# sanweiliti/LEMO

Hardware: AMD Instinct MI355X
Metric: fitting-iterations/sec (T=120 frames) (higher is better)
Workload: dtype f32

## Files before the change

lemo_amd/csrc/conv_pair_kernels.hip:

```cpp
#include "conv_common.hpp"
#include "conv_f16.hpp"

namespace lemo {

constexpr int CP_TH = 10, CP_TW = 14;
constexpr int CP_INW = CP_TW + 4, CP_INH = CP_TH + 4, CP_NIN = CP_INW * CP_INH;
constexpr int CP_MIDW = CP_TW + 2, CP_MIDH = CP_TH + 2, CP_NMID = CP_MIDW * CP_MIDH;
constexpr int CP_MIDP = CP_MIDW + 2, CP_NMIDP = CP_MIDP * CP_MIDH;
constexpr int CP_NOUT = CP_TH * CP_TW;
constexpr int CP_PL_IN = CP_NIN * 16, CP_GRP_IN = 2 * CP_PL_IN;
constexpr int CP_PL_MID = CP_NMIDP * 16, CP_GRP_MID = 2 * CP_PL_MID;
constexpr int CP_MID_OFF = 8 * CP_GRP_IN;
constexpr int CP_WMAX_OFF = CP_MID_OFF + 8 * CP_GRP_MID;
constexpr int CP_SMEM = CP_WMAX_OFF + 3 * 8 * 4;
constexpr int CP_NSLOT = 4;
static_assert(CP_MIDW == 16 && CP_NMID == 6 * 32 && CP_INW == CP_MIDP, "N-tiles = 2 rows x 16 columns on grids of row pitch 18");
static_assert(4 * 2 * CP_NIN <= CP_NSLOT * 512 && CP_NOUT == 140, "staging slots");
static_assert(8 * 6 * 256 * 4 <= CP_MID_OFF, "the K-half exchange (6 quads per wave) fits the dead input planes");

struct PairArgs {
  const float* in;
  const uint4* wA;
  const uint4* wB;
  const float *biasA, *biasB;
  const float *auxA, *auxB;
  float* mid;
  float* out;
  float winvA, winvB;
  int H, W, ntx, ntiles;
  unsigned long long* dbg;
};

template <int NT> struct PairSplit {
  static constexpr int NQ = NT == 3 ? 6 : 4;
  static constexpr int keep_tile(int KH, int i) { return i < 4 ? KH : 2; }
  static constexpr int keep_quad(int KH, int i) { return i < 4 ? i : (i - 4) + 2 * KH; }
  static constexpr int give_tile(int KH, int i) { return i < 4 ? 1 - KH : 2; }
  static constexpr int give_quad(int KH, int i) { return i < 4 ? i : (i - 4) + 2 * (1 - KH); }
};

template <int NT, int KH>
__device__ __forceinline__ void pair_exchange(const f32x16 (&acc)[3], float4 (&v)[6], float* red_mine, const float* red_theirs) {
  typedef PairSplit<NT> S;
#pragma unroll
  for (int i = 0; i < S::NQ; ++i) {
    const int t = S::give_tile(KH, i), q = S::give_quad(KH, i);
    st4(red_mine + i * 256, make_float4(acc[t][4 * q], acc[t][4 * q + 1], acc[t][4 * q + 2], acc[t][4 * q + 3]));
  }
  __syncthreads();
#pragma unroll
  for (int i = 0; i < S::NQ; ++i) {
    const int t = S::keep_tile(KH, i), q = S::keep_quad(KH, i);
    const float4 o = ld4(red_theirs + i * 256);
    const float4 m = make_float4(acc[t][4 * q], acc[t][4 * q + 1], acc[t][4 * q + 2], acc[t][4 * q + 3]);
    v[i] = KH ? make_float4(o.x + m.x, o.y + m.y, o.z + m.z, o.w + m.w) : make_float4(m.x + o.x, m.y + o.y, m.z + o.z, m.w + o.w);
  }
}

__device__ __forceinline__ int cp_lane_col(int j) { return j < 16 ? j : ((j - 18) & 15); }

#define CP_RA 3

__device__ __forceinline__ void pair_preload_a(uint4 (&ra)[CP_RA][2], const uint4* __restrict__ w, int kh, int ch, int lane) {
#pragma unroll
  for (int u0 = 0; u0 < CP_RA - 1; ++u0)
#pragma unroll
    for (int s_ = 0; s_ < 2; ++s_) ra[u0][s_] = w[(unsigned)((((2 * kh) * 9 + u0) * 2 + ch) * 2 + s_) * 64u + lane];
}

template <int NT, int GRP, int PL, int PITCH, typename MidFn, typename EndFn>
__device__ __forceinline__ void pair_kloop(f32x16 (&acc)[3], uint4 (&ra)[CP_RA][2], const uint4* __restrict__ w, const unsigned char* bbase,
                                           const int (&li)[3], int kh, int ch, int lane, MidFn&& mid_fn, EndFn&& end_fn) {
  const int h = lane >> 5;
  uint4 rb[2][3][2];
#define CP_LOAD_A(SET, U)                                                                              \
  _Pragma("unroll") for (int s_ = 0; s_ < 2; ++s_)                                                     \
    ra[SET][s_] = w[(unsigned)((((2 * kh + (U) / 9) * 9 + (U) % 9) * 2 + ch) * 2 + s_) * 64u + lane];
#define CP_LOAD_B(SET, U)                                                                              \
  _Pragma("unroll") for (int nt_ = 0; nt_ < NT; ++nt_)                                                 \
    _Pragma("unroll") for (int s_ = 0; s_ < 2; ++s_)                                                   \
      rb[SET][nt_][s_] = *reinterpret_cast<const uint4*>(                                              \
          bbase + (2 * (2 * kh + (U) / 9) + h) * GRP + s_ * PL + (li[nt_] + (((U) % 9) / 3 - 1) * PITCH + (((U) % 9) % 3 - 1)) * 16);
#define CP_MFMA1(SA, SETA, SB, SETB)                                                                   \
  _Pragma("unroll") for (int nt_ = 0; nt_ < NT; ++nt_)                                                 \
    acc[nt_] = __builtin_amdgcn_mfma_f32_32x32x16_f16(__builtin_bit_cast(f16x8, ra[SETA][SA]),         \
                                                      __builtin_bit_cast(f16x8, rb[SETB][nt_][SB]), acc[nt_], 0, 0, 0);
#pragma unroll
  for (int cc = 0; cc < 2; ++cc) {
    CP_LOAD_B((cc * 9) & 1, cc * 9)
#pragma unroll
    for (int tap = 0; tap < 9; ++tap) {
      const int u = cc * 9 + tap;
      if (u + CP_RA - 1 < 18) { CP_LOAD_A((u + CP_RA - 1) % CP_RA, u + CP_RA - 1) }
      if (tap + 1 < 9) { CP_LOAD_B((u + 1) & 1, u + 1) }
      __builtin_amdgcn_sched_barrier(0);
      CP_MFMA1(0, u % CP_RA, 1, u & 1) CP_MFMA1(1, u % CP_RA, 0, u & 1) CP_MFMA1(0, u % CP_RA, 0, u & 1)
      mid_fn(cc, tap);
      __builtin_amdgcn_sched_barrier(0);
    }
    end_fn(cc);
  }
#undef CP_LOAD_A
#undef CP_LOAD_B
#undef CP_MFMA1
}

template <int EPI, int NT>
__device__ __forceinline__ void pair_layer2(const PairArgs& a, unsigned char* smem, float* smem_f, int y0, int x0, int T0, int ng2, int ch,
                                            int kh, int lane, float smi, uint4 (&ra)[CP_RA][2]) {
  const int j = lane & 31, h = lane >> 5;
  const int Wp = a.W + 2, HWp = (a.H + 2) * Wp;
  int lo[3] = {0, 0, 0}, poff[3] = {0, 0, 0};
  bool ok[3] = {false, false, false};
#pragma unroll
  for (int nt = 0; nt < NT; ++nt) {
    const int oy = 2 * (T0 + nt) + (j >> 4), c = cp_lane_col(j), ox = c - 1;
    lo[nt] = (oy + 1) * CP_MIDP + c + 1;
    const int y = y0 + oy, x = x0 + ox;
    ok[nt] = ox >= 0 && ox < CP_TW && y < a.H && x < a.W;
    const int yc = y < a.H ? y : a.H - 1, xc = x < 0 ? 0 : (x < a.W ? x : a.W - 1);
    poff[nt] = (yc + 1) * Wp + (xc + 1);
  }
  f32x16 acc[3];
#pragma unroll
  for (int nt = 0; nt < 3; ++nt)
#pragma unroll
    for (int r = 0; r < 16; ++r) acc[nt][r] = 0.f;
  pair_kloop<NT, CP_GRP_MID, CP_PL_MID, CP_MIDP>(acc, ra, a.wB, smem + CP_MID_OFF, lo, kh, ch, lane, [](int, int) {}, [](int) {});
  {
    const float f = smi * a.winvB;
#pragma unroll
    for (int nt = 0; nt < NT; ++nt)
#pragma unroll
      for (int r = 0; r < 16; ++r) acc[nt][r] *= f;
  }
  typedef PairSplit<NT> S;
  const int KHu = __builtin_amdgcn_readfirstlane(kh);
  const int poA = KHu ? poff[1] : poff[0], poB = poff[2];
  const bool okA = KHu ? ok[1] : ok[0], okB = ok[2];
  float4 eo[6];
#pragma unroll
  for (int i = 0; i < S::NQ; ++i) {
    const int q = KHu ? S::keep_quad(1, i) : S::keep_quad(0, i);
    const int c0 = ch * 32 + q * 8 + 4 * h;
    const int po = i < 4 ? poA : poB;
    eo[i] = EPI == 1 ? ld4(a.auxB + ((size_t)(c0 >> 3) * HWp + po) * 8 + (c0 & 7)) : ld4(a.biasB + c0);
  }
  float* red = smem_f + ((ng2 * 2 + ch) * 2) * 1536 + lane * 4;
  float4 v[6];
  if (KHu) pair_exchange<NT, 1>(acc, v, red + 1536, red);
  else pair_exchange<NT, 0>(acc, v, red, red + 1536);
#pragma unroll
  for (int i = 0; i < S::NQ; ++i) {
    const int q = KHu ? S::keep_quad(1, i) : S::keep_quad(0, i);
    const int c0 = ch * 32 + q * 8 + 4 * h;
    const int po = i < 4 ? poA : poB;
    const bool st = i < 4 ? okA : okB;
    float4 r = v[i];
    if (EPI == 1) {
      r.x *= lrelu_grad_from_out(eo[i].x); r.y *= lrelu_grad_from_out(eo[i].y);
      r.z *= lrelu_grad_from_out(eo[i].z); r.w *= lrelu_grad_from_out(eo[i].w);
    } else {
      r.x = lrelu(r.x + eo[i].x); r.y = lrelu(r.y + eo[i].y); r.z = lrelu(r.z + eo[i].z); r.w = lrelu(r.w + eo[i].w);
    }
    if (st) st4(a.out + ((size_t)(c0 >> 3) * HWp + po) * 8 + (c0 & 7), r);
  }
}

template <int EPI, bool DBG>
__global__ void __launch_bounds__(512)
conv3x3_pair_kernel(PairArgs a) {
  unsigned long long t_start = 0, t_pro = 0, t_l1 = 0, t_mid = 0, t_ex = 0, t_mx = 0;
  if (DBG) t_start = __builtin_amdgcn_s_memtime();
  LEMO_DYN_SMEM(smem_f);
  unsigned char* smem = reinterpret_cast<unsigned char*>(smem_f);
  float* wmax = reinterpret_cast<float*>(smem + CP_WMAX_OFF);
  const int tid = (int)threadIdx.x, lane = tid & 63, wave = tid >> 6;
  const int j = lane & 31, h = lane >> 5;
  const int ng = wave & 1, ch = (wave >> 1) & 1, kh = wave >> 2;
  const int H = a.H, W = a.W, Wp = W + 2, HWp = (H + 2) * Wp;
  const unsigned in_gstride = (unsigned)HWp * 8u;
  int tile = (int)blockIdx.x;
  {
    const int q = a.ntiles >> 3, r = a.ntiles & 7, xcd = tile & 7, k = tile >> 3;
    tile = (xcd < r ? xcd * (q + 1) : r * (q + 1) + (xcd - r) * q) + k;
  }
  const int ty = tile / a.ntx, tx = tile - ty * a.ntx;
  const int y0 = ty * CP_TH, x0 = tx * CP_TW;

  uint4 ra[CP_RA][2];
  pair_preload_a(ra, a.wA, kh, ch, lane);

  unsigned offB[CP_NSLOT];
  int dstB[CP_NSLOT];
#pragma unroll
  for (int k = 0; k < CP_NSLOT; ++k) {
    int c0 = tid + k * 512;
    c0 = c0 < 4 * 2 * CP_NIN ? c0 : 4 * 2 * CP_NIN - 1;
    const int gg = c0 / (2 * CP_NIN), c = c0 - gg * (2 * CP_NIN);
    const int px = c >> 1, half = c & 1;
    const int r = px / CP_INW, col = px - r * CP_INW;
    int gy = y0 - 2 + r, gx = x0 - 2 + col;
    gy = (gy < -1 ? -1 : (gy > H ? H : gy)) + 1;
    gx = (gx < -1 ? -1 : (gx > W ? W : gx)) + 1;
    const int g0 = (gg >> 1) * 4 + (gg & 1);
    offB[k] = (unsigned)g0 * in_gstride + (unsigned)(gy * Wp + gx) * 8u + 4u * half;
    dstB[k] = g0 * CP_GRP_IN + px * 16 + 8 * half;
  }
  float4 stB[CP_NSLOT];
#pragma unroll
  for (int k = 0; k < CP_NSLOT; ++k) stB[k] = ld4(a.in + offB[k]);
  if (tid < CP_MIDH * 2 * 16) {
    const int pl = tid / (CP_MIDH * 2), rc = tid - pl * (CP_MIDH * 2);
    *reinterpret_cast<uint4*>(smem + CP_MID_OFF + pl * CP_PL_MID + ((rc >> 1) * CP_MIDP + (rc & 1) * (CP_MIDP - 1)) * 16) = make_uint4(0u, 0u, 0u, 0u);
  }
  float sc[2] = {1.f, 1.f}, sci[2] = {1.f, 1.f};
  {
    float m = 0.f;
#pragma unroll
    for (int k = 0; k < CP_NSLOT; ++k) m = absmax4(stB[k], m);
    m = wave_max(m);
    if (lane == 0) wmax[wave] = m;
    __syncthreads();
    float mm = 0.f;
#pragma unroll
    for (int i = 0; i < 8; ++i) mm = fmaxf(mm, wmax[i]);
    f16_scale_for(mm, sc[0], sci[0]);
  }
#pragma unroll
  for (int k = 0; k < CP_NSLOT; ++k) {
    uint2 s0, s1;
    split2x4(stB[k], sc[0], s0, s1);
    *reinterpret_cast<uint2*>(smem + dstB[k]) = s0;
    *reinterpret_cast<uint2*>(smem + dstB[k] + CP_PL_IN) = s1;
  }
#pragma unroll
  for (int k = 0; k < CP_NSLOT; ++k) stB[k] = ld4(a.in + 2u * in_gstride + offB[k]);
  __syncthreads();
  if (DBG) t_pro = __builtin_amdgcn_s_memtime();

  int li[3];
#pragma unroll
  for (int nt = 0; nt < 3; ++nt) {
    const int my = 2 * (3 * ng + nt) + (j >> 4), mx = cp_lane_col(j);
    li[nt] = (my + 1) * CP_INW + mx + 1;
  }
  f32x16 acc[3];
#pragma unroll
  for (int nt = 0; nt < 3; ++nt)
#pragma unroll
    for (int r = 0; r < 16; ++r) acc[nt][r] = 0.f;
  pair_kloop<3, CP_GRP_IN, CP_PL_IN, CP_INW>(
      acc, ra, a.wA, smem, li, kh, ch, lane,
      [&](int cc, int tap) {
        if (cc != 0) return;
        if (tap == 0) {
          float m = 0.f;
#pragma unroll
          for (int k = 0; k < CP_NSLOT; ++k) m = absmax4(stB[k], m);
          m = wave_max(m);
          if (lane == 0) wmax[8 + wave] = m;
        }
        if (tap == 1) {
          __syncthreads();
          float mm = 0.f;
#pragma unroll
          for (int i = 0; i < 8; ++i) mm = fmaxf(mm, wmax[8 + i]);
          f16_scale_after(mm, sc[0], sc[1], sci[1]);
        }
#pragma unroll
        for (int k = 0; k < CP_NSLOT; ++k) {
          if (2 + (7 * k) / CP_NSLOT != tap) continue;
          uint2 s0, s1;
          split2x4(stB[k], sc[1], s0, s1);
          *reinterpret_cast<uint2*>(smem + 2 * CP_GRP_IN + dstB[k]) = s0;
          *reinterpret_cast<uint2*>(smem + 2 * CP_GRP_IN + dstB[k] + CP_PL_IN) = s1;
        }
      },
      [&](int cc) {
        __syncthreads();
        if (cc == 0) {
          const float f = sc[1] * sci[0];
#pragma unroll
          for (int nt = 0; nt < 3; ++nt)
#pragma unroll
            for (int r = 0; r < 16; ++r) acc[nt][r] *= f;
        }
      });
  if (DBG) t_l1 = __builtin_amdgcn_s_memtime();
  pair_preload_a(ra, a.wB, kh, ch, lane);
  {
    const float f = sci[1] * a.winvA;
#pragma unroll
    for (int nt = 0; nt < 3; ++nt)
#pragma unroll
      for (int r = 0; r < 16; ++r) acc[nt][r] *= f;
  }

  const int KHu = __builtin_amdgcn_readfirstlane(kh);
  typedef PairSplit<3> S3;
  int mp0, mp1, mpoff0, mpoff1;
  bool inimg0, inimg1, inner0, inner1;
  {
    auto geom = [&](int t, int& p_, int& poff_, bool& inimg_, bool& inner_) {
      const int my = 2 * (3 * ng + t) + (j >> 4), mx = cp_lane_col(j);
      const int y = y0 - 1 + my, x = x0 - 1 + mx;
      p_ = my * CP_MIDP + mx + 1;
      inimg_ = (unsigned)y < (unsigned)H && (unsigned)x < (unsigned)W;
      inner_ = inimg_ && my >= 1 && my <= CP_TH && mx >= 1 && mx <= CP_TW;
      const int yc = y < 0 ? 0 : (y >= H ? H - 1 : y), xc = x < 0 ? 0 : (x >= W ? W - 1 : x);
      poff_ = (yc + 1) * Wp + (xc + 1);
    };
    geom(KHu, mp0, mpoff0, inimg0, inner0);
    geom(2, mp1, mpoff1, inimg1, inner1);
  }
  float4 eo[6];
#pragma unroll
  for (int i = 0; i < 6; ++i) {
    const int q = KHu ? S3::keep_quad(1, i) : S3::keep_quad(0, i);
    const int c0 = ch * 32 + q * 8 + 4 * h;
    const int po = i < 4 ? mpoff0 : mpoff1;
    eo[i] = EPI == 1 ? ld4(a.auxA + ((size_t)(c0 >> 3) * HWp + po) * 8 + (c0 & 7)) : ld4(a.biasA + c0);
  }
  float4 v[6];
  {
    float* red = smem_f + ((ng * 2 + ch) * 2) * 1536 + lane * 4;
    if (KHu) pair_exchange<3, 1>(acc, v, red + 1536, red);
    else pair_exchange<3, 0>(acc, v, red, red + 1536);
  }
  if (DBG) t_ex = __builtin_amdgcn_s_memtime();
  float mloc = 0.f;
#pragma unroll
  for (int i = 0; i < 6; ++i) {
    const bool in_i = i < 4 ? inimg0 : inimg1;
    float4 r = v[i];
    if (EPI == 1) {
      r.x *= lrelu_grad_from_out(eo[i].x); r.y *= lrelu_grad_from_out(eo[i].y);
      r.z *= lrelu_grad_from_out(eo[i].z); r.w *= lrelu_grad_from_out(eo[i].w);
    } else {
      r.x = lrelu(r.x + eo[i].x); r.y = lrelu(r.y + eo[i].y); r.z = lrelu(r.z + eo[i].z); r.w = lrelu(r.w + eo[i].w);
    }
    if (!in_i) r = make_float4(0.f, 0.f, 0.f, 0.f);
    v[i] = r;
    mloc = absmax4(r, mloc);
  }
  mloc = wave_max(mloc);
  if (lane == 0) wmax[16 + wave] = mloc;
  __syncthreads();
  float sm, smi;
  {
    float mm = 0.f;
#pragma unroll
    for (int i = 0; i < 8; ++i) mm = fmaxf(mm, wmax[16 + i]);
    f16_scale_for(mm, sm, smi);
  }
  if (DBG) t_mx = __builtin_amdgcn_s_memtime();
#pragma unroll
  for (int i = 0; i < 6; ++i) {
    const int q = KHu ? S3::keep_quad(1, i) : S3::keep_quad(0, i);
    uint2 s0, s1;
    split2x4(v[i], sm, s0, s1);
    unsigned char* d = smem + CP_MID_OFF + (ch * 4 + q) * CP_GRP_MID + (i < 4 ? mp0 : mp1) * 16 + 8 * h;
    *reinterpret_cast<uint2*>(d) = s0;
    *reinterpret_cast<uint2*>(d + CP_PL_MID) = s1;
  }
  __syncthreads();
  if (DBG) t_mid = __builtin_amdgcn_s_memtime();

  const int ng2 = __builtin_amdgcn_readfirstlane(ng ^ kh);
  if (ng2) pair_layer2<EPI, 2>(a, smem, smem_f, y0, x0, 3, 1, ch, kh, lane, smi, ra);
  else pair_layer2<EPI, 3>(a, smem, smem_f, y0, x0, 0, 0, ch, kh, lane, smi, ra);
  if (EPI != 1) {
#pragma unroll
    for (int i = 0; i < 6; ++i) {
      const int q = KHu ? S3::keep_quad(1, i) : S3::keep_quad(0, i);
      const int c0 = ch * 32 + q * 8 + 4 * h;
      if (i < 4 ? inner0 : inner1) st4(a.mid + ((size_t)(c0 >> 3) * HWp + (i < 4 ? mpoff0 : mpoff1)) * 8 + (c0 & 7), v[i]);
    }
  }
  if (DBG && lane == 0) {
    unsigned long long* r = a.dbg + ((size_t)blockIdx.x * 8 + wave) * 8;
    r[0] = __builtin_amdgcn_s_getreg(63492);
    r[1] = t_ex;
    r[2] = t_start; r[3] = __builtin_amdgcn_s_memtime(); r[4] = t_pro; r[5] = t_l1; r[6] = t_mid; r[7] = t_mx;
  }
}

int conv_pair_init() {
  static LdsOptinOnce once;
  return lds_optin(once, {{&conv3x3_pair_kernel<0, false>, CP_SMEM}, {&conv3x3_pair_kernel<1, false>, CP_SMEM}, {&conv3x3_pair_kernel<0, true>, CP_SMEM}});
}

bool conv3x3_pair_supported(int H, int W, int c0, int c1, int c2) {
  return c0 == 64 && c1 == 64 && c2 == 64 && H >= 1 && W >= 1 && (long)H * W <= (1l << 24);
}

int conv3x3_pair_f16(const float* in, const void* wA, float winvA, const float* biasA, const float* auxA, float* mid, const void* wB,
                     float winvB, const float* biasB, const float* auxB, float* out, int H, int W, int epi, hipStream_t s,
                     unsigned long long* dbg) {
  if (!conv3x3_pair_supported(H, W, 64, 64, 64) || (epi != 0 && epi != 1)) return LEMO_ERR_SHAPE;
  if (!in || !wA || !wB || !out || !(winvA > 0.f) || !(winvB > 0.f)) return LEMO_ERR_ARG;
  if (epi == 0 ? (!biasA || !biasB || !mid) : (!auxA || !auxB)) return LEMO_ERR_ARG;
  if (dbg && epi != 0) return LEMO_ERR_ARG;
  if (int rc = conv_pair_init()) return rc;
  PairArgs a{};
  a.in = in; a.wA = reinterpret_cast<const uint4*>(wA); a.wB = reinterpret_cast<const uint4*>(wB);
  a.biasA = biasA; a.biasB = biasB; a.auxA = auxA; a.auxB = auxB; a.mid = mid; a.out = out;
  a.winvA = winvA; a.winvB = winvB; a.H = H; a.W = W;
  a.ntx = (W + CP_TW - 1) / CP_TW;
  a.ntiles = a.ntx * ((H + CP_TH - 1) / CP_TH);
  a.dbg = dbg;
  if (dbg) hipLaunchKernelGGL((conv3x3_pair_kernel<0, true>), dim3(a.ntiles), dim3(512), CP_SMEM, s, a);
  else if (epi == 0) hipLaunchKernelGGL((conv3x3_pair_kernel<0, false>), dim3(a.ntiles), dim3(512), CP_SMEM, s, a);
  else hipLaunchKernelGGL((conv3x3_pair_kernel<1, false>), dim3(a.ntiles), dim3(512), CP_SMEM, s, a);
  return (int)hipGetLastError();
}

}
```

lemo_amd/priors.py:

```python
from __future__ import annotations

import ctypes as C
from typing import Dict, List

import numpy as np
import torch
import torch.nn as nn

from . import _hip
from ._hip import ptr

ENC_CHANNELS = [1, 32, 32, 64, 64, 64, 64, 64, 64, 64, 64]
"""models/AE_sep.py:77-89 with z_channel=64: channels before/after each of the 10 conv layers."""


def enc_layer_keys() -> List[str]:
    return [f'enc_blc{b}.main.{i}' for b in range(1, 6) for i in (0, 2)]


def pack_conv3x3(w: np.ndarray) -> np.ndarray:
    co, ci = w.shape[:2]
    assert ci % 8 == 0
    t = w.reshape(co, ci // 8, 8, 9)
    return np.ascontiguousarray(t.transpose(3, 1, 0, 2), np.float32)


def pack_conv3x3_bwd(w: np.ndarray) -> np.ndarray:
    wf = w[:, :, ::-1, ::-1].transpose(1, 0, 2, 3)
    return pack_conv3x3(np.ascontiguousarray(wf))


def pack_conv3x3_gmajor(w: np.ndarray) -> np.ndarray:
    return np.ascontiguousarray(pack_conv3x3(w).transpose(1, 0, 2, 3))


def pack_conv3x3_bwd_gmajor(w: np.ndarray) -> np.ndarray:
    return np.ascontiguousarray(pack_conv3x3_bwd(w).transpose(1, 0, 2, 3))


def bf16_round(x: np.ndarray) -> np.ndarray:
    u = np.ascontiguousarray(x, np.float32).view(np.uint32).astype(np.uint64)
    r = ((u + 0x7FFF + ((u >> 16) & 1)) >> 16) << 16
    return r.astype(np.uint32).view(np.float32)


def bf16_split3(x: np.ndarray):
    x = np.ascontiguousarray(x, np.float32)
    hi = bf16_round(x)
    r1 = x - hi
    mid = bf16_round(r1)
    lo = bf16_round(r1 - mid)
    assert np.array_equal(hi.astype(np.float64) + mid.astype(np.float64) + lo.astype(np.float64), x.astype(np.float64))
    return hi, mid, lo


def pack_conv3x3_split(w: np.ndarray) -> np.ndarray:
    co, ci = w.shape[:2]
    assert ci % 16 == 0 and co % 32 == 0
    pieces = np.stack(bf16_split3(w), 0)
    bits = (pieces.view(np.uint32) >> 16).astype(np.uint16)
    t = bits.reshape(3, co // 32, 32, ci // 16, 2, 8, 9)
    t = t.transpose(3, 6, 1, 0, 4, 2, 5)
    return np.ascontiguousarray(t).reshape(ci // 16, 9, co // 32, 3, 64, 8)


def pack_conv3x3_bwd_split(w: np.ndarray) -> np.ndarray:
    wf = w[:, :, ::-1, ::-1].transpose(1, 0, 2, 3)
    return pack_conv3x3_split(np.ascontiguousarray(wf))


def f16_split2(x: np.ndarray):
    x = np.ascontiguousarray(x, np.float32)
    m = float(np.abs(x).max())
    k = 14 - int(np.floor(np.log2(m))) if m > 0 else 0
    xs = x * np.float32(2.0 ** k)
    hi = xs.astype(np.float16)
    lo = (xs - hi.astype(np.float32)).astype(np.float16)
    assert np.isfinite(hi).all()
    return hi, lo, float(2.0 ** -k)


def pack_conv3x3_split_f16(w: np.ndarray):
    co, ci = w.shape[:2]
    assert ci % 16 == 0 and co % 32 == 0
    hi, lo, winv = f16_split2(w)
    bits = np.stack([hi, lo], 0).view(np.uint16)
    t = bits.reshape(2, co // 32, 32, ci // 16, 2, 8, 9)
    t = t.transpose(3, 6, 1, 0, 4, 2, 5)
    return np.ascontiguousarray(t).reshape(ci // 16, 9, co // 32, 2, 64, 8), winv


def pack_conv3x3_bwd_split_f16(w: np.ndarray):
    wf = w[:, :, ::-1, ::-1].transpose(1, 0, 2, 3)
    return pack_conv3x3_split_f16(np.ascontiguousarray(wf))


WINO_VARIANT = 10
_WINO_G = np.array([[1.0, 0.0, 0.0], [0.5, 0.5, 0.5], [0.5, -0.5, 0.5], [0.0, 0.0, 1.0]], np.float64)


def pack_conv3x3_wino_f16(w: np.ndarray):
    co, ci = w.shape[:2]
    assert co == 64 and ci == 64 and w.shape[2:] == (3, 3)
    U = np.einsum('ij,ocjk,lk->ocil', _WINO_G, np.asarray(w, np.float64), _WINO_G).reshape(co, ci, 16)
    m = float(np.abs(U).max())
    k = 14 - int(np.floor(np.log2(m))) if m > 0 else 0
    xs = U * 2.0 ** k
    hi = xs.astype(np.float16)
    lo = (xs - hi.astype(np.float64)).astype(np.float16)
    assert np.isfinite(hi).all()
    bits = np.stack([hi, lo], 0).view(np.uint16)
    t = bits.reshape(2, co // 32, 32, ci // 16, 2, 8, 16)
    t = t.transpose(6, 3, 1, 0, 4, 2, 5)
    return np.ascontiguousarray(t).reshape(16, ci // 16, co // 32, 2, 64, 8), float(2.0 ** -k)


def pack_conv3x3_bwd_wino_f16(w: np.ndarray):
    wf = w[:, :, ::-1, ::-1].transpose(1, 0, 2, 3)
    return pack_conv3x3_wino_f16(np.ascontiguousarray(wf))


def cg8p_alloc(C_: int, H: int, W: int, device) -> torch.Tensor:
    return torch.zeros(max(C_ // 8, 1), (H + 2) * (W + 2), 8, dtype=torch.float32, device=device)


def to_cg8p(x: torch.Tensor) -> torch.Tensor:
    Cn, H, W = x.shape
    buf = torch.zeros(Cn // 8, H + 2, W + 2, 8, dtype=torch.float32, device=x.device)
    buf[:, 1:-1, 1:-1, :] = x.reshape(Cn // 8, 8, H, W).permute(0, 2, 3, 1)
    return buf.reshape(Cn // 8, (H + 2) * (W + 2), 8).contiguous()


def from_cg8p(buf: torch.Tensor, H: int, W: int) -> torch.Tensor:
    G = buf.shape[0]
    return buf.reshape(G, H + 2, W + 2, 8)[:, 1:-1, 1:-1, :].permute(0, 3, 1, 2).reshape(G * 8, H, W).contiguous()


class EncWeights:

    def split_pack(self, l: int, bwd: bool, variant: int):
        if variant == WINO_VARIANT and self.w10[l] is not None:
            return (self.wbwd10[l], self.wbwd10_inv[l]) if bwd else (self.w10[l], self.w10_inv[l])
        if variant >= 4:
            return (self.wbwd4[l], self.wbwd4_inv[l]) if bwd else (self.w4[l], self.w4_inv[l])
        return ((self.wbwd3[l] if bwd else self.w3[l]), 1.0)

    def __init__(self, state: Dict[str, np.ndarray], device):
        self.keys = enc_layer_keys()
        t = lambda a: torch.from_numpy(np.ascontiguousarray(a, np.float32)).to(device)
        self.w, self.b, self.wbwd, self.w2, self.wbwd2 = [], [], [], [], []
        self.w3, self.wbwd3 = [], []
        self.w4, self.wbwd4, self.w4_inv, self.wbwd4_inv = [], [], [], []
        self.w10, self.wbwd10, self.w10_inv, self.wbwd10_inv = [], [], [], []
        t16 = lambda a: torch.from_numpy(a.view(np.int16)).to(device)
        for li, k in enumerate(self.keys):
            w = np.asarray(state[k + '.weight'], np.float32)
            b = np.asarray(state[k + '.bias'], np.float32)
            assert w.shape[0] == ENC_CHANNELS[li + 1] and w.shape[1] == ENC_CHANNELS[li], (k, w.shape)
            if li == 0:
                self.w.append(t(w.reshape(w.shape[0], 9)))
                self.wbwd.append(self.w[0])
                self.w2.append(self.w[0]); self.wbwd2.append(self.w[0])
                self.w3.append(None); self.wbwd3.append(None)
                self.w4.append(None); self.wbwd4.append(None); self.w4_inv.append(1.0); self.wbwd4_inv.append(1.0)
                self.w10.append(None); self.wbwd10.append(None); self.w10_inv.append(1.0); self.wbwd10_inv.append(1.0)
            else:
                self.w.append(t(pack_conv3x3(w)))
                self.wbwd.append(t(pack_conv3x3_bwd(w)))
                self.w2.append(t(pack_conv3x3_gmajor(w)))
                self.wbwd2.append(t(pack_conv3x3_bwd_gmajor(w)))
                self.w3.append(t16(pack_conv3x3_split(w)))
                self.wbwd3.append(t16(pack_conv3x3_bwd_split(w)))
                pf, fi = pack_conv3x3_split_f16(w)
                pb, bi = pack_conv3x3_bwd_split_f16(w)
                self.w4.append(t16(pf)); self.wbwd4.append(t16(pb)); self.w4_inv.append(fi); self.wbwd4_inv.append(bi)
                if w.shape[0] == 64 and w.shape[1] == 64:
                    uf, ufi = pack_conv3x3_wino_f16(w)
                    ub, ubi = pack_conv3x3_bwd_wino_f16(w)
                    self.w10.append(t16(uf)); self.wbwd10.append(t16(ub)); self.w10_inv.append(ufi); self.wbwd10_inv.append(ubi)
                else:
                    self.w10.append(None); self.wbwd10.append(None); self.w10_inv.append(1.0); self.wbwd10_inv.append(1.0)
            self.b.append(t(b))



DEFAULT_CONV_VARIANT = int(__import__('os').environ.get('LEMO_CONV_VARIANT', '9'))
"""Kernel family of the encoder's MFMA layers (``conv_variant`` of include/lemo_hip.h): 10 (round 6, selectable, measured slower: DESIGN 5) = 9 with every
64 -> 64 layer one Winograd F(2x2, 3x3) launch (csrc/conv_wino_kernels.hip) instead of the fused pairs; 9 (default since round 5) = 8 with layer 2's backward-data (64 -> 32) inside the
tail launch (+0.5 %); 8 = 7 with layer 2 (32 -> 64) inside the head launch as well (0 .. +0.9 % box to box); 7 = 5 plus the encoder's head and tail as one launch each (marker image + layers 0, 1 / their adjoints:
csrc/conv_head_kernels.hip, +2.1 % iterations/s); (6, the pairs on four-wave workgroups, was removed in round 6: csrc/attic); 5 = the engines run consecutive 64 -> 64
layers as fused PAIRS (one launch, intermediate in LDS; csrc/conv_pair_kernels.hip; the default since round 4) in the arithmetic
of 4 = split-f16 kernel (two error-compensated fp16 pieces per fp32 operand, 3 products; layer by layer -- what the module /
autograd path runs for 4 and 5 alike), 3 = split-bf16 kernel (three
exact bf16 pieces, 6 products), LDS-tiled fp32-MFMA kernel (2) for shapes they do not take; 2 / 1 = fp32 MFMA only.
The environment override exists for A/B runs of the parity suite."""


def check_conv_variant(v: int) -> int:
    v = int(v)
    if v == 6:
        raise ValueError('conv variant 6 (four-wave fused pairs) was removed in round 6: measured slower than variant 5 '
                         '(profiles/r05_pair4_check.txt); the source is in lemo_amd/csrc/attic')
    if v < 0 or v > WINO_VARIANT:
        raise ValueError(f'unknown conv variant {v}')
    return v


def _conv_layer(lib, enc: EncWeights, l: int, bwd: bool, x, out, aux, H, W, variant, s):
    cin, cout = (ENC_CHANNELS[l + 1], ENC_CHANNELS[l]) if bwd else (ENC_CHANNELS[l], ENC_CHANNELS[l + 1])
    wt, wt2, w3 = (enc.wbwd[l], enc.wbwd2[l], enc.wbwd3[l]) if bwd else (enc.w[l], enc.w2[l], enc.w3[l])
    bias, epi = (None, 1) if bwd else (ptr(enc.b[l]), 0)
    auxp = ptr(aux) if bwd else None
    if variant == WINO_VARIANT and enc.w10[l] is not None and lib.conv3x3_wino_supported(H, W, cin, cout):
        wu, winv = enc.split_pack(l, bwd, variant)
        lib.check(lib.conv3x3_wino_f16(ptr(x), ptr(wu), winv, ptr(wt), bias, auxp, ptr(out), H, W, epi, None, s), 'conv3x3_wino_f16')
    elif variant >= 4 and w3 is not None and lib.conv3x3_split_supported(H, W, cin, cout):
        w4, winv = enc.split_pack(l, bwd, 4)
        lib.check(lib.conv3x3_mfma_split_f16(ptr(x), ptr(w4), winv, ptr(wt), bias, auxp, ptr(out), H, W, cin, cout, epi, s), 'conv3x3_mfma_split_f16')
    elif variant >= 3 and w3 is not None and lib.conv3x3_split_supported(H, W, cin, cout):
        lib.check(lib.conv3x3_mfma_split(ptr(x), ptr(w3), ptr(wt), bias, auxp, ptr(out), H, W, cin, cout, epi, s), 'conv3x3_mfma_split')
    elif variant >= 2 and 127 + 2 * (127 // W + 1) + 2 * (W + 2) + 3 <= 416:
        lib.check(lib.conv3x3_mfma_lds(ptr(x), ptr(wt), ptr(wt2), bias, auxp, ptr(out), H, W, cin, cout, epi, s), 'conv3x3_mfma_lds')
    else:
        lib.check(lib.conv3x3_mfma(ptr(x), ptr(wt), bias, auxp, ptr(out), H, W, cin, cout, epi, 1, s), 'conv3x3_mfma')


def _enc_forward(lib, enc: EncWeights, x: torch.Tensor, variant: int = None):
    H, W = x.shape
    dev = x.device
    s = lib.stream(dev)
    variant = DEFAULT_CONV_VARIANT if variant is None else variant
    x0 = torch.zeros(H + 2, W + 2, dtype=torch.float32, device=dev)
    x0[1:-1, 1:-1] = x
    act = [x0] + [cg8p_alloc(ENC_CHANNELS[l], H, W, dev) for l in range(1, 11)]
    lib.check(lib.conv3x3_c1(ptr(x0), ptr(enc.w[0]), ptr(enc.b[0]), ptr(act[1]), H, W, ENC_CHANNELS[1], s), 'conv3x3_c1')
    for l in range(1, 10):
        _conv_layer(lib, enc, l, False, act[l], act[l + 1], None, H, W, variant, s)
    return act, variant


def _enc_backward(lib, enc: EncWeights, act, dpre10: torch.Tensor, variant: int) -> torch.Tensor:
    H, W = act[0].shape[0] - 2, act[0].shape[1] - 2
    dev = dpre10.device
    s = lib.stream(dev)
    cur, other = dpre10, cg8p_alloc(64, H, W, dev)
    for l in range(9, 0, -1):
        _conv_layer(lib, enc, l, True, cur, other, act[l], H, W, variant, s)
        cur, other = other, cur
    dx = torch.empty(H, W, dtype=torch.float32, device=dev)
    lib.check(lib.conv3x3_c1_bwd(ptr(cur), ptr(enc.w[0]), ptr(dx), H, W, ENC_CHANNELS[1], s), 'conv3x3_c1_bwd')
    return dx


class _SmoothPriorLoss(torch.autograd.Function):

    @staticmethod
    def forward(ctx, x, enc: EncWeights, lib):
        x = x.contiguous().float()
        _hip.check_device(lib, x)
        H, W = x.shape
        act, use_lds = _enc_forward(lib, enc, x)
        cnt = 64 * H * (W - 1)
        nb = lib.smooth_loss_blocks(H, W, 64)
        part = torch.zeros(nb, dtype=torch.float32, device=x.device)
        dpre = cg8p_alloc(64, H, W, x.device)
        lib.check(lib.smooth_loss(ptr(act[10]), ptr(dpre), ptr(part), H, W, 64, 2.0 / cnt, lib.stream(x.device)), 'smooth_loss')
        ctx.enc, ctx.lib, ctx.act, ctx.dpre, ctx.use_lds = enc, lib, act, dpre, use_lds
        return (part.double().sum() / cnt).float()

    @staticmethod
    def backward(ctx, g):
        dx = _enc_backward(ctx.lib, ctx.enc, ctx.act, ctx.dpre, ctx.use_lds)
        return dx * g, None, None


class _EncFn(torch.autograd.Function):

    @staticmethod
    def forward(ctx, x, enc: EncWeights, lib):
        x = x.contiguous().float()
        _hip.check_device(lib, x)
        act, use_lds = _enc_forward(lib, enc, x)
        ctx.enc, ctx.lib, ctx.act, ctx.use_lds = enc, lib, act, use_lds
        H, W = x.shape
        return from_cg8p(act[10], H, W)

    @staticmethod
    def backward(ctx, dz):
        H, W = dz.shape[1:]
        dz = dz.contiguous().float()
        z = from_cg8p(ctx.act[10], H, W)
        dpre = to_cg8p(dz * torch.where(z > 0, 1.0, 0.2))
        return _enc_backward(ctx.lib, ctx.enc, ctx.act, dpre, ctx.use_lds), None, None


class _Conv3x3Param(nn.Module):

    def __init__(self, cin, cout):
        super().__init__()
        self.weight = nn.Parameter(torch.zeros(cout, cin, 3, 3))
        self.bias = nn.Parameter(torch.zeros(cout))


class _EncBlockParams(nn.Module):
    def __init__(self, cin, cout):
        super().__init__()
        self.main = nn.ModuleDict({'0': _Conv3x3Param(cin, cout), '2': _Conv3x3Param(cout, cout)})


class Enc(nn.Module):

    def __init__(self, downsample=False, z_channel=64, _lib=None):
        super().__init__()
        if downsample or z_channel != 64:
            raise NotImplementedError('LEMO instantiates the smoothness encoder as Enc(downsample=False, z_channel=64)')
        ch = ENC_CHANNELS
        for b in range(1, 6):
            setattr(self, f'enc_blc{b}', _EncBlockParams(ch[2 * b - 2], ch[2 * b]))
        self._lib_override, self._cache = _lib, {}

    def packed(self, device) -> EncWeights:
        ps = list(self.parameters())
        key = (str(device),) + tuple((p.data_ptr(), p._version) for p in ps)
        if self._cache.get('key') != key:
            sd = {k: v.detach().cpu().numpy() for k, v in self.state_dict().items()}
            self._cache = dict(key=key, enc=EncWeights(sd, device))
        return self._cache['enc']

    def forward(self, x):
        assert x.dim() == 4 and x.shape[0] == 1 and x.shape[1] == 1, 'the fitting path feeds [1,1,d,T] clips'
        lib = self._lib_override or _hip.get_lib()
        z = _EncFn.apply(x[0, 0], self.packed(x.device), lib)
        sz = lambda c: torch.Size([1, c, x.shape[2], x.shape[3]])
        return z.unsqueeze(0), x.size(), sz(32), sz(64), sz(64), sz(64)

    def smooth_loss(self, x):
        lib = self._lib_override or _hip.get_lib()
        return _SmoothPriorLoss.apply(x[0, 0], self.packed(x.device), lib)


def warn_if_wide_image(lib, H: int, W: int, conv_variant: int) -> bool:
    import warnings
    H, W = int(H), int(W)
    too_wide = 127 + 2 * (127 // W + 1) + 2 * (W + 2) + 3 > 408
    if conv_variant >= 3 and H * W >= 128 and too_wide and not lib.conv3x3_split_supported(H, W, 64, 64):
        warnings.warn(f'lemo_amd: smoothness image {H} x {W} is wider than the split-f16 single-layer kernels take (W <= 134, i.e. clips of '
                      f'up to 120 frames); the 32-channel layers and the unpaired 64 -> 64 layers run on the slower fp32-input kernels',
                      RuntimeWarning, stacklevel=3)
        return True
    return False



DEC_IN = [64, 64, 64, 64, 64, 64, 64, 32, 32, 1]
DEC_OUT = [64, 64, 64, 64, 64, 64, 32, 32, 1, 1]
"""models/AE_sep.py:102-122 with downsample=False, z_channel=64: (nin, nout) of the 10 stride-1 transposed convolutions."""


def dec_layer_keys() -> List[str]:
    return [f'dec_blc{b}.deconv{i}' for b in range(1, 6) for i in (1, 2)]


class _DeconvParam(nn.Module):

    def __init__(self, nin, nout):
        super().__init__()
        self.weight = nn.Parameter(torch.zeros(nin, nout, 3, 3))
        self.bias = nn.Parameter(torch.zeros(nout))


class _DecBlockParams(nn.Module):
    def __init__(self, nin, nout):
        super().__init__()
        self.deconv1 = _DeconvParam(nin, nout)
        self.deconv2 = _DeconvParam(nout, nout)


class Dec(nn.Module):

    def __init__(self, downsample=False, z_channel=64, _lib=None):
        super().__init__()
        if downsample or z_channel != 64:
            raise NotImplementedError('LEMO instantiates the smoothness decoder as Dec(downsample=False, z_channel=64)')
        for b in range(1, 6):
            setattr(self, f'dec_blc{b}', _DecBlockParams(DEC_IN[2 * b - 2], DEC_OUT[2 * b - 2]))
        self._lib_override, self._cache = _lib, {}

    def packed(self, device):
        ps = list(self.parameters())
        key = (str(device),) + tuple((p.data_ptr(), p._version) for p in ps)
        if self._cache.get('key') != key:
            sd = {k: v.detach().cpu().numpy().astype(np.float32) for k, v in self.state_dict().items()}
            t = lambda a: torch.from_numpy(np.ascontiguousarray(a, np.float32)).to(device)
            wt, wt2, bias = [], [], []
            for j, k in enumerate(dec_layer_keys()):
                w = sd[k + '.weight']
                assert w.shape == (DEC_IN[j], DEC_OUT[j], 3, 3), (k, w.shape)
                if j < 8:
                    wt.append(t(pack_conv3x3_bwd(w))); wt2.append(t(pack_conv3x3_bwd_gmajor(w)))
                else:
                    wt.append(t(w.reshape(DEC_IN[j], 9))); wt2.append(None)
                bias.append(t(sd[k + '.bias']))
            self._cache = dict(key=key, packs=(wt, wt2, bias))
        return self._cache['packs']

    def forward(self, z, input_size=None, s1=None, s2=None, s3=None, s4=None):
        assert z.dim() == 4 and z.shape[1] == 64, 'z: [bs, 64, H, W]'
        lib = self._lib_override or _hip.get_lib()
        z = z.detach().contiguous().float()
        _hip.check_device(lib, z)
        bs, _, H, W = z.shape
        dev = z.device
        s = lib.stream(dev)
        wt, wt2, bias = self.packed(dev)
        cur = [to_cg8p(z[b]) for b in range(bs)]
        for j in range(8):
            nxt = [cg8p_alloc(64, H, W, dev) for _ in range(bs)]
            for b in range(bs):
                lib.check(lib.conv3x3_mfma_lds(ptr(cur[b]), ptr(wt[j]), ptr(wt2[j]), ptr(bias[j]), None, ptr(nxt[b]), H, W,
                                               DEC_IN[j], DEC_OUT[j], 0, s), 'conv3x3_mfma_lds')
            cur = nxt
        u = torch.stack(cur)
        r1 = torch.zeros(bs, H + 2, W + 2, dtype=torch.float32, device=dev)
        rec = torch.zeros_like(r1)
        lib.check(lib.dec_end_fwd(ptr(u), u[0].numel(), ptr(wt[8]), ptr(bias[8]), ptr(wt[9]), ptr(bias[9]), ptr(r1), ptr(rec),
                                  bs, H, W, s), 'dec_end_fwd')
        return rec[:, 1:-1, 1:-1].unsqueeze(1).contiguous()
```

Baseline: 3217.

## Derive mid-layer f16 scale from weight L1 bound instead of block-wide max reduction

Replaces the post-activation block-wide absmax reduction (wave_max, shared-memory write, __syncthreads, and a read of 8 values) with an a-priori bound. The bound is the input absmax times the layer-A weight row L1 norm plus the max bias magnitude. The L1 bound is computed on the host and appended as a tail to the packed weight array. This removes one barrier and its reduction from the fused pair kernel, but the scale can be looser than the true max, which may cost f16 split precision in the intermediate activations.

```diff
diff --git a/lemo_amd/csrc/conv_pair_kernels.hip b/lemo_amd/csrc/conv_pair_kernels.hip
--- a/lemo_amd/csrc/conv_pair_kernels.hip
+++ b/lemo_amd/csrc/conv_pair_kernels.hip
@@ -12,7 +12,8 @@
 constexpr int CP_PL_MID = CP_NMIDP * 16, CP_GRP_MID = 2 * CP_PL_MID;
 constexpr int CP_MID_OFF = 8 * CP_GRP_IN;
 constexpr int CP_WMAX_OFF = CP_MID_OFF + 8 * CP_GRP_MID;
-constexpr int CP_SMEM = CP_WMAX_OFF + 3 * 8 * 4;
+constexpr int CP_SMEM = CP_WMAX_OFF + 2 * 8 * 4;
+constexpr int CP_WTAIL = 4 * 9 * 2 * 2 * 64;
 constexpr int CP_NSLOT = 4;
 static_assert(CP_MIDW == 16 && CP_NMID == 6 * 32 && CP_INW == CP_MIDP, "N-tiles = 2 rows x 16 columns on grids of row pitch 18");
 static_assert(4 * 2 * CP_NIN <= CP_NSLOT * 512 && CP_NOUT == 140, "staging slots");
@@ -190,6 +191,8 @@
 
   uint4 ra[CP_RA][2];
   pair_preload_a(ra, a.wA, kh, ch, lane);
+  const float l1A = __builtin_bit_cast(float, a.wA[CP_WTAIL].x);
+  float bmax = EPI == 0 ? fabsf(a.biasA[lane]) : 0.f;
 
   unsigned offB[CP_NSLOT];
   int dstB[CP_NSLOT];
@@ -215,6 +218,7 @@
     *reinterpret_cast<uint4*>(smem + CP_MID_OFF + pl * CP_PL_MID + ((rc >> 1) * CP_MIDP + (rc & 1) * (CP_MIDP - 1)) * 16) = make_uint4(0u, 0u, 0u, 0u);
   }
   float sc[2] = {1.f, 1.f}, sci[2] = {1.f, 1.f};
+  float min_;
   {
     float m = 0.f;
 #pragma unroll
@@ -226,6 +230,7 @@
 #pragma unroll
     for (int i = 0; i < 8; ++i) mm = fmaxf(mm, wmax[i]);
     f16_scale_for(mm, sc[0], sci[0]);
+    min_ = mm;
   }
 #pragma unroll
   for (int k = 0; k < CP_NSLOT; ++k) {
@@ -267,6 +272,7 @@
 #pragma unroll
           for (int i = 0; i < 8; ++i) mm = fmaxf(mm, wmax[8 + i]);
           f16_scale_after(mm, sc[0], sc[1], sci[1]);
+          min_ = fmaxf(min_, mm);
         }
 #pragma unroll
         for (int k = 0; k < CP_NSLOT; ++k) {
@@ -289,6 +295,9 @@
       });
   if (DBG) t_l1 = __builtin_amdgcn_s_memtime();
   pair_preload_a(ra, a.wB, kh, ch, lane);
+  float sm, smi;
+  if (EPI == 0) bmax = wave_max(bmax);
+  f16_scale_for(fmaf(min_, l1A, bmax), sm, smi);
   {
     const float f = sci[1] * a.winvA;
 #pragma unroll
@@ -329,7 +338,6 @@
     else pair_exchange<3, 0>(acc, v, red, red + 1536);
   }
   if (DBG) t_ex = __builtin_amdgcn_s_memtime();
-  float mloc = 0.f;
 #pragma unroll
   for (int i = 0; i < 6; ++i) {
     const bool in_i = i < 4 ? inimg0 : inimg1;
@@ -342,17 +350,6 @@
     }
     if (!in_i) r = make_float4(0.f, 0.f, 0.f, 0.f);
     v[i] = r;
-    mloc = absmax4(r, mloc);
-  }
-  mloc = wave_max(mloc);
-  if (lane == 0) wmax[16 + wave] = mloc;
-  __syncthreads();
-  float sm, smi;
-  {
-    float mm = 0.f;
-#pragma unroll
-    for (int i = 0; i < 8; ++i) mm = fmaxf(mm, wmax[16 + i]);
-    f16_scale_for(mm, sm, smi);
   }
   if (DBG) t_mx = __builtin_amdgcn_s_memtime();
 #pragma unroll
diff --git a/lemo_amd/priors.py b/lemo_amd/priors.py
--- a/lemo_amd/priors.py
+++ b/lemo_amd/priors.py
@@ -80,6 +80,27 @@
     return hi, lo, float(2.0 ** -k)
 
 
+def conv3x3_l1_bound(w: np.ndarray) -> np.float32:
+    v = float(np.abs(np.asarray(w, np.float64)).reshape(w.shape[0], -1).sum(1).max()) * (1.0 + 2.0 ** -10)
+    f = np.float32(v)
+    return f if float(f) >= v else np.nextafter(f, np.float32(np.inf))
+
+
+def pair_mid_bound_binades(x: torch.Tensor, mid: torch.Tensor, l1: float, bmax: float = 0.0) -> torch.Tensor:
+    TH, TW = 10, 14
+    H, W = x.shape[-2:]
+    nty, ntx = -(-H // TH), -(-W // TW)
+
+    def tile_max(a, halo):
+        a = a.abs().amax(0)[None, None].double()
+        a = torch.nn.functional.pad(a, (halo, (ntx - 1) * TW + TW + halo - W, halo, (nty - 1) * TH + TH + halo - H))
+        return torch.nn.functional.max_pool2d(a, (TH + 2 * halo, TW + 2 * halo), (TH, TW))[0, 0]
+    bound = (tile_max(x, 2).float() * np.float32(l1) + np.float32(bmax)).double()
+    m = tile_max(mid, 1)
+    keep = m > 0
+    return torch.floor(torch.log2(bound[keep])) - torch.floor(torch.log2(m[keep]))
+
+
 def pack_conv3x3_split_f16(w: np.ndarray):
     co, ci = w.shape[:2]
     assert ci % 16 == 0 and co % 32 == 0
@@ -87,7 +108,8 @@
     bits = np.stack([hi, lo], 0).view(np.uint16)
     t = bits.reshape(2, co // 32, 32, ci // 16, 2, 8, 9)
     t = t.transpose(3, 6, 1, 0, 4, 2, 5)
-    return np.ascontiguousarray(t).reshape(ci // 16, 9, co // 32, 2, 64, 8), winv
+    tail = np.array([conv3x3_l1_bound(w), 0, 0, 0], np.float32).view(np.uint16)
+    return np.concatenate([np.ascontiguousarray(t).reshape(-1), tail]), winv
 
 
 def pack_conv3x3_bwd_split_f16(w: np.ndarray):
```

Result: no change. 3231, median of 6 (+0.5%).
